# zrc0622/HIRL4UCAV

Measured on AMD Instinct MI355X. Metric: env steps/sec (whole node) + HIRL update steps/sec at 4096 envs/GPU, higher is better.
Workload: dtype f32

## Files before the change

hirl4ucav_amd/agents/engine.py:

```python
import ctypes
import os

import numpy as np
import torch

from .. import _lib

H1, H2 = 256, 512
_vp, _i32, _f32 = ctypes.c_void_p, ctypes.c_int32, ctypes.c_float


class HxBatch(ctypes.Structure):
    _fields_ = [("rows", _vp), ("bc_rows", _vp), ("batch", _i32), ("noise", _vp)]


class HxSample(ctypes.Structure):
    _fields_ = [("total", _vp), ("cap", ctypes.c_int64), ("ring", _vp), ("expert_ring", _vp), ("expert_len", ctypes.c_int64),
                ("bc_table", _vp), ("bc_len", ctypes.c_int64), ("n_main", _i32), ("seed", ctypes.c_uint64), ("call", ctypes.c_uint32),
                ("sigma", _f32), ("idx", _vp), ("idx_bc", _vp), ("guard", ctypes.c_uint32)]


class HxFront(ctypes.Structure):
    _fields_ = [("flags", _vp), ("status", _vp), ("epoch", ctypes.c_uint32), ("with_c", ctypes.c_uint32)]

# ... 415 lines not shown
        B, st = self.batch, _lib.stream_ptr()
        nets, hyper = ctypes.byref(self.nets), ctypes.byref(self.hyper)
        gs = 1.0 / self.world
        own_critic = self.grad_critic.data_ptr()
        if self.xchg is not None:
            self.nets.grad_critic = self.xchg.write_buffer("critic").data_ptr()
        critic_grads()
        if before_exchange is not None:
            before_exchange()
        summed = self._allreduce(self.grad_critic, "critic")
        self.nets.grad_critic = summed.data_ptr()
        pk = 16 if do_polyak else 0
        _lib.call("hx_adam", nets, hyper, 0 | pk, self.critic_step, gs, 0, 0.0, 0.0, B, st)
        self.nets.grad_critic = own_critic
        if actor_phase:
            _lib.call("hx_hirl_actor_backward", nets, ctypes.byref(batch), hyper, int(w_kind == 1), 1, st)
            if self.world > 1 or self.sharded_sequence:
                if self.actor_msg is None:
                    self.actor_msg = torch.zeros(int(_lib.load().hx_actor_message_floats()), dtype=torch.float32, device=self.device)
                msg = self.xchg.write_buffer("actor") if self.xchg is not None else self.actor_msg
                _lib.call("hx_hirl_actor_wgrad_split", nets, hyper, B, msg.data_ptr(), st)
                summed = self._allreduce(msg, "actor")
                _lib.call("hx_adam_mixed", nets, hyper, int(do_polyak), self.actor_step, gs, w_kind, w_given, float(bc_warm_up_weight),
                          B * self.world, summed.data_ptr(), st)
            else:
                _lib.call("hx_hirl_actor_wgrad", nets, hyper, B, B, w_kind, w_given, float(bc_warm_up_weight), st)
                _lib.call("hx_adam", nets, hyper, 1 | pk, self.actor_step, gs, w_kind, w_given, float(bc_warm_up_weight), B, st)

    def step_learn(self, env, expert=None, bc_table=None, n_main=None, act_noise=None, act_sigma=0.0, act_seed=0, out=None, sample_seed=0,
                   smooth_sigma=0.2, bc_weight_now=0.0, bc_warm_up_weight=0.0):
        replay, n, B = env.replay, env.n, self.batch
# ... 68 lines not shown
        knob = os.environ.get("HX_FRONT_C")
        carries_c = knob == "1" or (bool(with_c) and knob != "0")
        if carries_c:
            self._front_c_epoch += 1
        front = HxFront(flags.data_ptr(), status.data_ptr(), self._front_epoch, self._front_c_epoch if carries_c else 0)
        _lib.call("hx_hirl_front", env.state.data_ptr(), n, env.pitch, env.obs.data_ptr(), out.data_ptr(), mode | (32 if (not bf16 and self._x9_for(n, front=True)) else 0),
                  _lib.ptr(act_noise), float(act_sigma), int(act_seed), int(env.env_id0), self.act_calls, env.reward.data_ptr(), env.done.data_ptr(),
                  env.success.data_ptr(), ctypes.byref(env._opts), nets, ctypes.byref(batch), hyper, int(actor_phase), w_kind, ctypes.byref(front), st)
        self._front_enqueued = True
        env.steps_issued += 1
        nxt_draw, nxt_tiles = draw(nxt, self.sample_calls + 1), tiles_of(nxt)
        if not self.staged:
            _lib.call("hx_hirl_learn_back", nets, ctypes.byref(batch), hyper, self.critic_step, int(actor_phase), self.actor_step, int(do_polyak), w_kind, w_given,
                      float(bc_warm_up_weight), ctypes.byref(nxt_draw), ctypes.byref(nxt_tiles), with_c, st)
        else:
            self._learn_staged(lambda: _lib.call("hx_hirl_critic_grads_back", nets, ctypes.byref(batch), hyper, ctypes.byref(nxt_draw), ctypes.byref(nxt_tiles), with_c, st),
                               batch, actor_phase, do_polyak, w_kind, w_given, bc_warm_up_weight)
        self._front_drawn = (env, env.steps_issued, replay, expert, bc_table, n_main, int(sample_seed), float(smooth_sigma), self.sample_calls + 1, n)
        self._front_tiles = [nxt, cur]
        self.rows, self.bc_rows, self._idx, self._idx_bc, self._noise = cur
        self.actor_trainable = not self.actor_trainable
        return out, env.obs, env.reward, env.done, env.success

    @staticmethod
    def front_waiting_workgroups(batch, with_c=False):
        tiles = (int(batch) + 15) // 16
        return 2 * tiles * 8 + (2 * ((int(batch) + 7) // 8) * 8 if with_c else 0)

    def front_c_for(self, n, actor_phase, w_kind, bf16):
        if self.front_c != "auto":
            return bool(self.front_c)
# ... 34 lines not shown
```

hirl4ucav_amd/csrc/hx_fwd_body.h:

```cpp
#pragma once
#include "hx_update.h"

namespace hxu {

struct FwdJobC {
    const float* net; const float* src; const float* noise; const float* prev_net;
    float* ws; float* prev_ws;
    uint32_t cfg;
    int32_t rows;
    float noise_clamp;
    float slope;
};
static_assert(sizeof(FwdJobC) == 64, "one s_load_dwordx16");
struct FwdArgsC {
    FwdJobC job[6];
    float slope;
    int zero_nf;
    float* zero_f;
    int* zero_i;
    const uint16_t* images;
    int rowmap;
};
inline FwdJobC pack_fwd(const FwdJob& J) {
    FwdJobC c{};
// ... 72 lines not shown
    const int in = J.m.in;
    constexpr int TPC = WIDE ? 16 : kWide / NT;
    constexpr int NW2 = WIDE ? 1 : H1 / (TPC * 4);
    v4f w2v[NW2];
    uint4 bq[BF16 ? NSL : 1];
    const int lr = lane & 15, lg = lane >> 4, u = wave * 16 + lr;
    STAMP_DECL;
    STAMP();
    const float4* W1v = reinterpret_cast<const float4*>(J.net + J.m.W1());
    const int n4 = H1 * in / 4;
    const float4 wv0 = tid < n4 ? W1v[tid] : make_float4(0.f, 0.f, 0.f, 0.f);
    const float4 wv1 = tid + kWide < n4 ? W1v[tid + kWide] : make_float4(0.f, 0.f, 0.f, 0.f);
    const float bias1 = J.net[J.m.b1() + u], g1v = J.net[J.m.g1() + u], be1v = J.net[J.m.be1() + u];
    const float bias2 = J.net[J.m.b2() + nt * NTW + (WIDE ? wave * 16 : (wave % CT) * 16) + (lane & 15)];
    const int xr = tid / XP, xc = tid % XP;
    const bool head_mode = in == 17 && J.act_mode != 0 && J.act_mode != 3;
    float xv = 0.0f;
    float4 tile_piece = make_float4(0.f, 0.f, 0.f, 0.f);
    if constexpr (SAMPLE) {
        draw_fused(SA, J.rows, s_hkey, s_hown, s_fin);
        if (tid < RT * XP && xr < nrow) {
            const int r = r0 + xr;
            const float* row = (r < SA.n_main ? SA.ring : SA.expert_ring) + (size_t)s_fin[0][r] * 32;
            if (xc < 13) xv = row[J.col0 + xc];
            else if (in == 17 && xc < 17 && J.act_mode == 0) xv = row[xc];
        }
        if (by == 0 && nt < 2 && tid < nrow * 8) {
            const int r = r0 + (tid >> 3);
            if (nt == 0) tile_piece = reinterpret_cast<const float4*>((r < SA.n_main ? SA.ring : SA.expert_ring) + (size_t)s_fin[0][r] * 32)[tid & 7];
            else if (SA.bc_rows) tile_piece = reinterpret_cast<const float4*>(SA.bc_table + (size_t)s_fin[1][r] * 32)[tid & 7];
        }
    } else if (tid < RT * XP && xr < nrow) {
        if (xc < 13) xv = src_row(J.src, r0 + xr)[J.col0 + xc];
        else if (in == 17 && xc < 17) {
            if (J.act_mode == 0) xv = src_row(J.src, r0 + xr)[xc];
            else if (J.act_mode == 3) xv = J.noise[(size_t)(r0 + xr) * 4 + (xc - 13)];
        }
    }
    if constexpr (BF16) {
        const int ctile = WIDE ? nt * 16 + wave : nt * CT + wave % CT;
        const int sl0 = WIDE ? 0 : (wave / CT) * NSL;
        const uint16_t* blk = A.images + (size_t)J.img * kImgElems + (size_t)(ctile * 8 + sl0) * 512 + lane * 8;
#pragma unroll
        for (int i = 0; i < NSL; ++i) bq[i] = *reinterpret_cast<const uint4*>(blk + i * 512);
    } else if (!WIDE) {
        const float* wcol = J.net + J.m.W2() + (size_t)(nt * NT + tid / TPC) * H1 + (tid % TPC) * 4;
#pragma unroll
        for (int i = 0; i < NW2; ++i) w2v[i] = *reinterpret_cast<const v4f*>(wcol + i * TPC * 4);
    }
    STAMP();
    if constexpr (FRONT == 2) {
// ... 1 lines not shown
            if (tid == 0) {
                int spins = 0;
                while ((int)(__hip_atomic_load(&X.flags[rt], __ATOMIC_RELAXED, __HIP_MEMORY_SCOPE_AGENT) - X.target) < 0) {
                    if (++spins > 4000000) { atomicOr(X.status, 1u); break; }
                    __builtin_amdgcn_s_sleep(1);
                }
            }
            __syncthreads();
            if (tid < nrow * 4) xs[(tid >> 2) * XP + 13 + (tid & 3)] = ld_agent(J.prev.ws.outv + (size_t)(r0 + (tid >> 2)) * OW + (tid & 3));
        }
    }
    if (FRONT != 2 && head_mode && wave < nrow) {
        const int r = wave;
        RowReg<H2> xh, y;
        float mean, rstd, o[4];
        if (J.prev.m.out == 4) head_row4<RELU>(J.prev.ws.z2 + (size_t)(r0 + r) * H2, J.prev.net, J.prev.m, slope, xh, y, mean, rstd, o);
        else head_row<4, RELU>(J.prev.ws.z2 + (size_t)(r0 + r) * H2, J.prev.net, J.prev.m, slope, xh, y, mean, rstd, o);
        if (lane < 4) {
            float a = fast_tanh(lane == 0 ? o[0] : lane == 1 ? o[1] : lane == 2 ? o[2] : o[3]);
            if (J.noise) {
                const float e = fminf(fmaxf(J.noise[lane], -J.noise_clamp), J.noise_clamp);
                a = fminf(fmaxf(a + e, -1.0f), 1.0f);
            }
            xs[r * XP + 13 + lane] = a;
            if (nt == 0) J.prev.ws.outv[(size_t)(r0 + r) * OW + lane] = a;
        }
        if (nt == 0 && lane == 0) {
            J.prev.ws.st2[(size_t)(r0 + r) * 2] = mean;
            J.prev.ws.st2[(size_t)(r0 + r) * 2 + 1] = rstd;
        }
    }
// ... 161 lines not shown
            if (tid == 0) __hip_atomic_fetch_add(&X.flags[(FRONT == 1 ? 16 * by : 48) + rt], 1u, __ATOMIC_RELAXED, __HIP_MEMORY_SCOPE_AGENT);
        }
    }
    if constexpr (FRONT == 1) {
        if (by == 0) {
            __builtin_amdgcn_s_waitcnt(0);
            __syncthreads();
            int* last = reinterpret_cast<int*>(lds);
            if (tid == 0) *last = __hip_atomic_fetch_add(&X.flags[rt], 1u, __ATOMIC_RELAXED, __HIP_MEMORY_SCOPE_AGENT) + 1u == X.arrive;
            __syncthreads();
            if (*last) {
                if (wave < nrow) {
                    const int r = wave;
                    RowReg<H2> xh, y;
                    float mean, rstd, o[4];
                    if (J.m.out == 4) head_row4<RELU, true>(J.ws.z2 + (size_t)(r0 + r) * H2, J.net, J.m, slope, xh, y, mean, rstd, o);
                    else head_row<4, RELU, true>(J.ws.z2 + (size_t)(r0 + r) * H2, J.net, J.m, slope, xh, y, mean, rstd, o);
                    if (lane < 4) {
                        float a = fast_tanh(lane == 0 ? o[0] : lane == 1 ? o[1] : lane == 2 ? o[2] : o[3]);
                        if (X.noise) {
                            const float e = fminf(fmaxf(X.noise[lane], -X.noise_clamp), X.noise_clamp);
                            a = fminf(fmaxf(a + e, -1.0f), 1.0f);
                        }
                        st_agent(&J.ws.outv[(size_t)(r0 + r) * OW + lane], a);
                    }
                    if (lane == 0) {
                        J.ws.st2[(size_t)(r0 + r) * 2] = mean;
                        J.ws.st2[(size_t)(r0 + r) * 2 + 1] = rstd;
                    }
                }
                __builtin_amdgcn_s_waitcnt(0);
// ... 13 lines not shown
```

hirl4ucav_amd/csrc/hx_hirl.hip:

```cpp
#include <cmath>

#include "hx_act.h"

using namespace hxnn;
using namespace hxu;

extern "C" {

int hx_actor_param_count(void) { return kActor.size(); }
int hx_critic_param_count(void) { return 2 * kQ.padded(); }
int64_t hx_hirl_workspace_floats(int32_t batch) { return (int64_t)S_COUNT * kSlotFloats * batch + 64; }
int64_t hx_actor_message_floats(void) { return 2 * (int64_t)kActor.padded() + 64; }
int64_t hx_bf16_images_elems(void) { return (int64_t)IM_COUNT * (int64_t)kImgElems; }

int hx_pack_update_images(const HxNets* N, void* stream) {
    HX_REQUIRE(N && N->w2_bf16_all && (reinterpret_cast<uintptr_t>(N->w2_bf16_all) & 15u) == 0, "hx_pack_update_images: w2_bf16_all must be a 16-byte aligned buffer");
    HX_REQUIRE(N->actor && N->critic && N->target_actor && N->target_critic, "hx_pack_update_images: null network");
    hipStream_t st = (hipStream_t)stream;
    uint16_t* im = N->w2_bf16_all;
    launch_pack_bf16(N->actor + kActor.W2(), im + IM_ACTOR * kImgElems, false, st);
    launch_pack_bf16(N->actor + kActor.W2(), im + IM_ACTOR_T * kImgElems, true, st);
    launch_pack_bf16(N->target_actor + kActor.W2(), im + IM_TA * kImgElems, false, st);
    if (N->bc_actor) launch_pack_bf16(N->bc_actor + kActor.W2(), im + IM_BC * kImgElems, false, st);
    for (int h = 0; h < 2; ++h) {
// ... 72 lines not shown
    G = BwdArgs{};
    G.njobs = 2; G.slope = Hy->slope; G.inv_batch = 1.0f / B; G.losses = N->losses; G.soft_count = N->soft_count;
    for (int h = 0; h < 2; ++h) {
        BwdJob& J = G.job[h];
        J = BwdJob{};
        J.net = N->critic + h * mQ.padded(); J.m = mQ; J.ws = s[S_C1 + h]; J.rows = B; J.mode = BM_CRITIC_TD;
        J.t1 = Head{tc1, mQ, s[S_TC1]}; J.t2 = Head{tc2, mQ, s[S_TC2]}; J.src = src; J.gamma = Hy->gamma;
        J.img_t = IM_C1_T + h;
    }
    G.images = N->w2_bf16_all;
}
static bool front_has_c(bool asked) {
    static const int force = getenv("HX_FRONT_C") ? atoi(getenv("HX_FRONT_C")) : -1;
    return force < 0 ? asked : force != 0;
}
static int critic_back(const HxNets* N, const HxBatch* Bt, const HxHyper* Hy, void* stream, int adam_step, bool polyak, const SampleDev* predraw = nullptr, bool skip_c = false) {
    hipStream_t st = (hipStream_t)stream;
    const Mlp mQ{17, 1, Hy->no_layernorm ? 1 : 0};
    const int B = Bt->batch;
    Slot s[S_COUNT];
    make_slots(N, B, s);
    if (!skip_c) {
        BwdArgs G;
        make_launch_c(N, Bt, Hy, G);
        launch_bwd(0, G, st);
    }
    {
        WgArgs W{};
        W.njobs = 2; W.slope = Hy->slope; W.w_kind = 0; W.w_given = 0.f; W.inv_batch = 1.0f / B;
        W.soft_count = N->soft_count; W.wstate = N->wstate;
        for (int h = 0; h < 2; ++h) {
            WgJob& J = W.job[h];
            J = WgJob{};
            J.net = N->critic + h * mQ.padded(); J.grad = N->grad_critic + h * mQ.padded(); J.m = mQ;
            J.ws[0] = s[S_C1 + h]; J.rows[0] = B; J.nslots = 1; J.wmode[0] = 0;
            if (adam_step > 0) {
                J.p = N->critic + h * mQ.padded();
                J.mom = N->m_critic + h * mQ.padded(); J.var = N->v_critic + h * mQ.padded();
                J.target = polyak ? N->target_critic + h * mQ.padded() : nullptr;
                if (uint16_t* im = N->w2_bf16_all) {
                    J.w2b = im + (IM_C1 + h) * kImgElems; J.w2tb = im + (IM_C1_T + h) * kImgElems; J.tgt_w2b = im + (IM_TC1 + h) * kImgElems;
                }
            }
        }
        W.bf16 = N->w2_bf16_all != nullptr;
        W.predraw = predraw; W.predraw_batch = B;
        if (adam_step > 0) {
            W.ad = make_adam(N, Hy, Hy->lr_critic, adam_step, false);
            launch_wg(W, true, st);
        } else {
            launch_wg(W, false, st);
        }
    }
    HX_CHECK_LAUNCH("hx_hirl_critic_grads");
    return 0;
}
static int critic_grads_impl(const HxNets* N, const HxBatch* Bt, const HxHyper* Hy, int32_t actor_fwd, void* stream, int adam_step, bool polyak,
                             const HxSample* S = nullptr) {
    HX_REQUIRE(N && Bt && Hy && Bt->batch > 0 && Bt->batch % 16 == 0, "hx_hirl_critic_grads: batch must be a positive multiple of 16");
    hipStream_t st = (hipStream_t)stream;
    const int B = Bt->batch;
    SampleDev SD{};
    bool fused = false;
    if (S) {
        HX_REQUIRE(Bt->noise, "hx_hirl_*_sampled: the draw needs the output word noise[4]");
        if (int rc = prepare_draw(S, B, const_cast<float*>(Bt->rows), const_cast<float*>(Bt->bc_rows), const_cast<float*>(Bt->noise), stream, &SD, &fused)) return rc;
    }
    FwdArgs F;
    make_launch_a(N, Bt, Hy, actor_fwd, F);
    F.sample = fused ? &SD : nullptr;
    launch_fwd(F, st);
    make_launch_b(N, Bt, Hy, actor_fwd, F);
    launch_fwd(F, st);
    return critic_back(N, Bt, Hy, stream, adam_step, polyak);
}
int hx_hirl_critic_grads(const HxNets* N, const HxBatch* Bt, const HxHyper* Hy, int32_t actor_fwd, void* stream) {
    return critic_grads_impl(N, Bt, Hy, actor_fwd, stream, 0, false);
}
int hx_hirl_critic_grads_sampled(const HxNets* N, const HxBatch* Bt, const HxHyper* Hy, const HxSample* S, int32_t actor_fwd, void* stream) {
    HX_REQUIRE(S, "hx_hirl_critic_grads_sampled: null sample description");
    return critic_grads_impl(N, Bt, Hy, actor_fwd, stream, 0, false, S);
}

int hx_hirl_actor_backward(const HxNets* N, const HxBatch* Bt, const HxHyper* Hy, int32_t estimate_soft, int32_t fwd_done, void* stream) {
    HX_REQUIRE(N && Bt && Hy && Bt->batch > 0 && Bt->batch % 16 == 0, "hx_hirl_actor_backward: batch must be a positive multiple of 16");
    hipStream_t st = (hipStream_t)stream;
    const Mlp mA{13, 4, Hy->no_layernorm ? 1 : 0}, mQ{17, 1, Hy->no_layernorm ? 1 : 0};
    (void)mA; (void)mQ;
    const int B = Bt->batch;
    Slot s[S_COUNT];
    make_slots(N, B, s);
    const RowSrc src{Bt->rows, nullptr, nullptr, 0, 32};
    const RowSrc bcsrc{Bt->bc_rows ? Bt->bc_rows : Bt->rows, nullptr, nullptr, 0, 32};
    const bool bc = Hy->use_bc != 0, soft = bc && estimate_soft;
    if (!fwd_done) {
        FwdArgs F{};
        F.slope = Hy->slope;
        F.zero_f = N->losses + 1; F.zero_nf = 4; F.zero_i = N->soft_count;
        int n = 0;
        F.job[n++] = FwdJob{N->actor, mA, src, 0, 0, Head{}, nullptr, 0.f, s[S_API], B, 1, IM_ACTOR};
        if (bc) F.job[n++] = FwdJob{N->actor, mA, bcsrc, 0, 0, Head{}, nullptr, 0.f, s[S_ABC], B, 1, IM_ACTOR};
        if (soft) F.job[n++] = FwdJob{N->bc_actor, mA, src, 0, 0, Head{}, nullptr, 0.f, s[S_BCS], B, 0, IM_BC};
        F.njobs = n;
        F.images = N->w2_bf16_all;
        launch_fwd(F, st);
    }
    {
        FwdArgs F{};
        F.slope = Hy->slope;
        int n = 0;
        F.job[n++] = FwdJob{N->critic, mQ, src, 0, 1, Head{N->actor, mA, s[S_API]}, nullptr, 0.f, s[S_CPI], B, 1, IM_C1};
        if (soft) F.job[n++] = FwdJob{N->critic, mQ, src, 0, 1, Head{N->bc_actor, mA, s[S_BCS]}, nullptr, 0.f, s[S_CSOFT], B, 0, IM_C1};
        F.njobs = n;
        F.images = N->w2_bf16_all;
        launch_fwd(F, st);
    }
    {
        BwdArgs G{};
        G.njobs = 1; G.slope = Hy->slope; G.inv_batch = 1.0f / B; G.losses = N->losses; G.soft_count = N->soft_count;
        BwdJob& J = G.job[0];
        J = BwdJob{};
        J.net = N->critic; J.m = mQ; J.ws = s[S_CPI]; J.rows = B; J.mode = BM_CRITIC_PI;
        if (soft) J.soft = Head{N->critic, mQ, s[S_CSOFT]};
        J.img_t = IM_C1_T;
        G.images = N->w2_bf16_all;
        launch_bwd(1, G, st);
    }
// ... 88 lines not shown
    W.count_out = msg + 2 * mA.padded();
    launch_wg(W, false, (hipStream_t)stream);
    HX_CHECK_LAUNCH("hx_hirl_actor_wgrad_split");
    return 0;
}

int hx_hirl_learn(const HxNets* N, const HxBatch* Bt, const HxHyper* Hy, int32_t critic_step, int32_t actor_phase,
                  int32_t actor_step, int32_t do_polyak, int32_t w_kind, float w_given, float warm, void* stream) {
    return hx_hirl_learn_sampled(N, Bt, Hy, nullptr, critic_step, actor_phase, actor_step, do_polyak, w_kind, w_given, warm, stream);
}
int hx_hirl_learn_sampled(const HxNets* N, const HxBatch* Bt, const HxHyper* Hy, const HxSample* S, int32_t critic_step, int32_t actor_phase,
                          int32_t actor_step, int32_t do_polyak, int32_t w_kind, float w_given, float warm, void* stream) {
    HX_REQUIRE(critic_step >= 1 && (!actor_phase || actor_step >= 1), "hx_hirl_learn: Adam steps are 1-based");
    int rc = critic_grads_impl(N, Bt, Hy, actor_phase ? (w_kind == 1 ? 2 : 1) : 0, stream, critic_step, do_polyak != 0, S);
    if (rc || !actor_phase) return rc;
    if ((rc = hx_hirl_actor_backward(N, Bt, Hy, w_kind == 1, 1, stream))) return rc;
    return actor_wgrad_impl(N, Hy, Bt->batch, Bt->batch, w_kind, w_given, warm, stream, actor_step, do_polyak != 0);
}

int hx_hirl_front(float* state, int64_t n, int64_t stride, float* obs_io, float* actions, int32_t noise_mode, const float* noise,
                  float sigma, uint64_t seed, uint32_t row0, uint32_t call, float* reward, uint8_t* done, int8_t* success, const HxStepOpts* opts,
                  const HxNets* N, const HxBatch* Bt, const HxHyper* Hy, int32_t actor_phase, int32_t w_kind, const HxFront* front, void* stream) {
    HX_REQUIRE(N && Bt && Hy && front && opts && Bt->batch > 0 && Bt->batch % 16 == 0 && Bt->batch <= kFusedBatchMax && Bt->rows && Bt->noise,
               "hx_hirl_front: the minibatch tiles (a positive multiple of 16 rows, at most 256) and noise[4] must be there");
    HX_REQUIRE(front->flags && front->status && front->epoch >= 1, "hx_hirl_front: flags, status and a 1-based epoch are required");
    const bool bf16 = N->w2_bf16_all != nullptr;
    HX_REQUIRE(bf16 ? N->actor_w2_bf16 != nullptr : (!N->actor_w2_bf16 && (N->actor_w2_f32i || N->actor_w2_x9)),
               "hx_hirl_front: fp32 networks with HxNets.actor_w2_f32i / actor_w2_x9, or the bf16 update path (w2_bf16_all) with actor_w2_bf16");
    const int actor_fwd = actor_phase ? (w_kind == 1 ? 2 : 1) : 0;
    FwdArgs FA, FB;
    make_launch_a(N, Bt, Hy, actor_fwd, FA);
// ... 13 lines not shown
                        *front, (hipStream_t)stream);
}
static int make_predraw(const HxNets* N, const HxBatch* Bt, const HxSample* next, const HxBatch* next_tiles, void* stream, SampleDev* SD) {
    HX_REQUIRE(next_tiles && next_tiles->batch == Bt->batch && next_tiles->rows && next_tiles->noise && next_tiles->rows != Bt->rows && next_tiles->noise != Bt->noise,
               "hx_hirl_learn_back: the next minibatch needs tiles of its own (this call still reads the current ones)");
    (void)N;
    bool fused = false;
    if (int rc = prepare_draw(next, Bt->batch, const_cast<float*>(next_tiles->rows), const_cast<float*>(next_tiles->bc_rows), const_cast<float*>(next_tiles->noise),
                              stream, SD, &fused, false)) return rc;
    HX_REQUIRE(fused, "hx_hirl_learn_back: the predraw covers minibatches of at most 256 rows");
    return 0;
}
int hx_hirl_critic_grads_back(const HxNets* N, const HxBatch* Bt, const HxHyper* Hy, const HxSample* next, const HxBatch* next_tiles, int32_t c_in_front,
                              void* stream) {
    HX_REQUIRE(N && Bt && Hy && Bt->batch > 0 && Bt->batch % 16 == 0, "hx_hirl_critic_grads_back: batch must be a positive multiple of 16");
    SampleDev SD{};
    if (next) if (int rc = make_predraw(N, Bt, next, next_tiles, stream, &SD)) return rc;
    return critic_back(N, Bt, Hy, stream, 0, false, next ? &SD : nullptr, front_has_c(c_in_front != 0));
}
int hx_hirl_learn_back(const HxNets* N, const HxBatch* Bt, const HxHyper* Hy, int32_t critic_step, int32_t actor_phase, int32_t actor_step, int32_t do_polyak,
                       int32_t w_kind, float w_given, float warm, const HxSample* next, const HxBatch* next_tiles, int32_t c_in_front, void* stream) {
    HX_REQUIRE(N && Bt && Hy && Bt->batch > 0 && Bt->batch % 16 == 0, "hx_hirl_learn_back: batch must be a positive multiple of 16");
    HX_REQUIRE(critic_step >= 1 && (!actor_phase || actor_step >= 1), "hx_hirl_learn_back: Adam steps are 1-based");
    SampleDev SD{};
    if (next) if (int rc = make_predraw(N, Bt, next, next_tiles, stream, &SD)) return rc;
    int rc = critic_back(N, Bt, Hy, stream, critic_step, do_polyak != 0, next ? &SD : nullptr, front_has_c(c_in_front != 0));
    if (rc || !actor_phase) return rc;
    if ((rc = hx_hirl_actor_backward(N, Bt, Hy, w_kind == 1, 1, stream))) return rc;
    return actor_wgrad_impl(N, Hy, Bt->batch, Bt->batch, w_kind, w_given, warm, stream, actor_step, do_polyak != 0);
}

int hx_bc_train_actor(const HxNets* N, const HxBatch* Bt, const HxHyper* Hy, int32_t step, void* stream) {
    HX_REQUIRE(N && Bt && Hy && Bt->bc_rows && Bt->batch > 0 && Bt->batch % 16 == 0 && step >= 1, "hx_bc_train_actor: bad arguments");
    hipStream_t st = (hipStream_t)stream;
    const Mlp mA{13, 4, Hy->no_layernorm ? 1 : 0}, mQ{17, 1, Hy->no_layernorm ? 1 : 0};
    (void)mA; (void)mQ;
    const int B = Bt->batch;
    Slot s[S_COUNT];
    make_slots(N, B, s);
    const RowSrc bcsrc{Bt->bc_rows, nullptr, nullptr, 0, 32};
    {
        FwdArgs F{};
        F.njobs = 1; F.slope = Hy->slope;
// ... 31 lines not shown
```

hirl4ucav_amd/csrc/hx_update.h:

```cpp
#pragma once
#include <cmath>
#include <cstdlib>
#include <type_traits>

#include "hx_common.h"
#include "hx_nn.h"

#ifdef HX_STAMPS
static __device__ float hx_dbg[80];
#define STAMP_DECL unsigned long long TS_[16]; int tsn_ = 0
#define STAMP() TS_[tsn_++] = __builtin_amdgcn_s_memrealtime()
#define STAMP_FLUSH(base, cond) do { if (cond) { for (int i_ = 1; i_ < tsn_; ++i_) hx_dbg[(base) + i_] = (float)(TS_[i_] - TS_[i_ - 1]); hx_dbg[(base)] = (float)tsn_; } } while (0)
constexpr int kSpanCap = 8192;
static __device__ unsigned long long hx_span[kSpanCap][2];
static __device__ unsigned hx_span_tag[kSpanCap];
static __device__ unsigned hx_span_n;
#define SPAN_LOG(tag) do { if (threadIdx.x == 0) { const unsigned long long e_ = __builtin_amdgcn_s_memrealtime(); const unsigned i_ = atomicAdd(&hx_span_n, 1u); \
    if (i_ < (unsigned)kSpanCap) { hx_span[i_][0] = TS_[0]; hx_span[i_][1] = e_; hx_span_tag[i_] = (unsigned)(tag) | (blockIdx.x << 8) | (blockIdx.y << 24); } } } while (0)
#define HX_DEFINE_DEBUG_COLLECTORS(name, lo, hi) \
    namespace hx { \
    int dbg_stamps_##name(float* host80) { \
        float tmp[80]; \
        if (hipMemcpyFromSymbol(tmp, HIP_SYMBOL(hx_dbg), sizeof(tmp)) != hipSuccess) return -2; \
        for (int i = (lo); i < (hi); ++i) host80[i] = tmp[i]; \
// ... 127 lines not shown
    }
#pragma unroll
    for (int j = 0; j < OUTMAX; ++j) {
        float acc = 0.0f;
        if (j < m.out) {
            RowReg<H2> w;
            w.load(net + m.W3() + j * H2);
#pragma unroll
            for (int i = 0; i < 8; ++i) acc += act_f<RELU>(y.v[i], slope) * w.v[i];
            acc = wave_sum(acc) + net[m.b3() + j];
        }
        o[j] = acc;
    }
}

template <bool RELU, bool AGENT = false>
__device__ __forceinline__ void head_row4(const float* __restrict__ z2row, const float* __restrict__ net, const Mlp m, float slope,
                                          RowReg<H2>& xhat, RowReg<H2>& y, float& mean, float& rstd, float (&o)[4]) {
    RowReg<H2> z, g, be, w0, w1, w2, w3;
    if (AGENT) z.load_agent(z2row);
    else z.load(z2row);
    g.load(net + m.g2());
    be.load(net + m.be2());
    w0.load(net + m.W3());
    w1.load(net + m.W3() + H2);
    w2.load(net + m.W3() + 2 * H2);
    w3.load(net + m.W3() + 3 * H2);
    const int lane = threadIdx.x & 63;
    const float b3 = net[m.b3() + (lane & 3)];
    row_stats<8>(z.v, H2, mean, rstd);
    if (m.no_ln) { mean = 0.0f; rstd = 1.0f; }
    float a0 = 0.f, a1 = 0.f, a2 = 0.f, a3 = 0.f;
#pragma unroll
    for (int i = 0; i < 8; ++i) {
        xhat.v[i] = (z.v[i] - mean) * rstd;
        y.v[i] = g.v[i] * xhat.v[i] + be.v[i];
    }
#pragma unroll
    for (int i = 0; i < 8; ++i) a0 += act_f<RELU>(y.v[i], slope) * w0.v[i];
#pragma unroll
    for (int i = 0; i < 8; ++i) a1 += act_f<RELU>(y.v[i], slope) * w1.v[i];
#pragma unroll
    for (int i = 0; i < 8; ++i) a2 += act_f<RELU>(y.v[i], slope) * w2.v[i];
#pragma unroll
    for (int i = 0; i < 8; ++i) a3 += act_f<RELU>(y.v[i], slope) * w3.v[i];
    o[0] = wave_sum(a0) + __shfl(b3, 0);
    o[1] = wave_sum(a1) + __shfl(b3, 1);
    o[2] = wave_sum(a2) + __shfl(b3, 2);
    o[3] = wave_sum(a3) + __shfl(b3, 3);
}

__device__ __forceinline__ void philox4x32_10(uint32_t c0, uint32_t c1, uint32_t c2, uint32_t c3, uint32_t k0, uint32_t k1, uint32_t out[4]) {
#pragma unroll
    for (int r = 0; r < 10; ++r) {
        const uint32_t h0 = __umulhi(0xD2511F53u, c0), l0 = 0xD2511F53u * c0;
        const uint32_t h1 = __umulhi(0xCD9E8D57u, c2), l1 = 0xCD9E8D57u * c2;
        const uint32_t n0 = h1 ^ c1 ^ k0, n2 = h0 ^ c3 ^ k1;
        c0 = n0; c1 = l1; c2 = n2; c3 = l0;
        k0 += 0x9E3779B9u; k1 += 0xBB67AE85u;
    }
// ... 330 lines not shown
    float target_entropy, alpha_step_size;
};
struct WgArgs {
    WgJob job[2];
    int njobs;
    float slope;
    WgAdam ad;
    int w_kind;
    float w_given, warm, inv_batch;
    const int* soft_count;
    const float* wstate;
    int bf16;
    float* count_out;
    const SampleDev* predraw;
    int predraw_batch;
};

#pragma clang fp contract(off)
__device__ __forceinline__ void adam_update(float& p, float& m, float& v, float g, float b1, float b2, float eps, float step_size, float bc2_sqrt) {
    m = __builtin_fmaf(g, 1.0f - b1, m * b1);
    v = __builtin_fmaf(g * g, 1.0f - b2, v * b2);
    const float denom = __builtin_amdgcn_sqrtf(v) * __builtin_amdgcn_rcpf(bc2_sqrt) + eps;
    p = p - step_size * (m * __builtin_amdgcn_rcpf(denom));
}
__device__ __forceinline__ float polyak_update(float target, float p, float tau) { return target * (1.0f - tau) + p * tau; }
#pragma clang fp contract(fast)
__device__ __forceinline__ void sac_alpha_step(float* alpha_state, float* losses, float mean_h, float te, float b1, float b2, float eps, float step_size,
                                               float bc2_sqrt) {
    float la = alpha_state[0], m = alpha_state[1], v = alpha_state[2];
    losses[3] = -(la * (te - mean_h));
    adam_update(la, m, v, mean_h - te, b1, b2, eps, step_size, bc2_sqrt);
// ... 202 lines not shown
```

hirl4ucav_amd/csrc/hx_wgrad.hip:

```cpp
#include <cmath>

#include "hx_update.h"

using namespace hxnn;
using namespace hxu;

namespace {

struct WgJobC {
    const float* net; float* grad;
    float* ws0; float* ws1;
    float* mom; float* var; float* target; uint16_t* w2b; float* w2f;
    uint32_t cfg;
    int32_t rows0, rows1;
    float slope, w_given, warm, inv_batch;
    float b1, b2, eps, step_size, bc2_sqrt, tau;
    uint32_t pad_;
    const int* soft_count; float* wstate; float* losses;
    uint16_t* w2tb; uint16_t* tgt_w2b;
    float* count_out;
};
static_assert(sizeof(WgJobC) == 176, "WgJobC layout");
struct WgArgsC {
    WgJobC job[2];
    int has_pre, pre_batch;
    SampleDev pre;
};

struct AdamElem {
    float p, m, v, t;
    __device__ __forceinline__ void fetch(const WgJob& J, unsigned idx) {
        p = J.p[idx];
        m = J.mom[idx];
        v = J.var[idx];
        t = J.target ? J.target[idx] : 0.0f;
    }
    __device__ __forceinline__ void apply(const WgJob& J, const WgAdam& a, unsigned idx, float g) {
        adam_update(p, m, v, g, a.b1, a.b2, a.eps, a.step_size, a.bc2_sqrt);
        J.p[idx] = p;
// ... 169 lines not shown
    const float xh = (z - ri.x) * ri.y;
    const float dy = act_bwd<RELU>(d, g1 * xh + be1, slope);
    const float dz = sc * (ri.y * (dy * g1 - ri.z - xh * ri.w));
    a.db1 += dz;
    a.dbe += sc * dy;
    a.dg += sc * dy * xh;
    const float4* xr4 = reinterpret_cast<const float4*>(xrow);
#pragma unroll
    for (int q = 0; q < 4; ++q) {
        const float4 x4 = xr4[q];
        a.dw1[4 * q] += dz * x4.x; a.dw1[4 * q + 1] += dz * x4.y; a.dw1[4 * q + 2] += dz * x4.z; a.dw1[4 * q + 3] += dz * x4.w;
    }
    a.dw1[16] += dz * xrow[16];
}

#ifdef HX_STAMPS_L1
#define STAMP_L1() STAMP()
#else
#define STAMP_L1()
#endif
template <bool ADAM, bool RELU, bool BF16 = false>
__global__ __launch_bounds__(kWide) void wgrad_kernel(WgArgsC AC) {
    __shared__ __attribute__((aligned(16))) float lds[kWgRowChunk * XP + kWgRowChunk * 12 + kWgRG * kWgCols * kRedP];
    float* xs = lds;
    float* rinfo = lds + kWgRowChunk * XP;
    float* red = rinfo + kWgRowChunk * 12;

    {
        static_assert(sizeof(lds) >= (4 * kFusedSlots + 2 * kFusedBatchMax) * 4, "predraw_wg's tables fit");
        if (AC.has_pre && blockIdx.x >= kWgPerJob) {
            if (blockIdx.x == kWgPerJob && blockIdx.y == 0) predraw_wg(AC.pre, AC.pre_batch, lds);
            return;
        }
    }
    const int j = blockIdx.y, b = blockIdx.x;
    WgJob J;
    WgArgs A;
    expand_wg(AC.job[j], J, A);
    const int tid = threadIdx.x, wave = tid >> 6, lane = tid & 63;
    const float slope = A.slope;
    STAMP_DECL;
    STAMP();
    const float w = effective_w(A.w_kind, A.w_given, A.warm, A.inv_batch, A.soft_count, A.wstate);
    float scale[2];
#pragma unroll
    for (int s = 0; s < 2; ++s) scale[s] = J.wmode[s] == 0 ? 1.0f : (J.wmode[s] == 1 ? 1.0f - w : w);
// ... 568 lines not shown
        const float4 s4 = *reinterpret_cast<const float4*>(source + i);
        t4.x = polyak_update(t4.x, s4.x, tau);
        t4.y = polyak_update(t4.y, s4.y, tau);
        t4.z = polyak_update(t4.z, s4.z, tau);
        t4.w = polyak_update(t4.w, s4.w, tau);
        *reinterpret_cast<float4*>(target + i) = t4;
        return;
    }
    for (int c = 0; c < n - i; ++c) target[i + c] = polyak_update(target[i + c], source[i + c], tau);
}

}

namespace hxu {

void launch_wg(const WgArgs& W, bool adam, hipStream_t st) {
    WgArgsC C{};
    for (int j = 0; j < W.njobs; ++j) C.job[j] = pack_wg(W.job[j], W);
    const bool pre = W.predraw != nullptr;
    C.has_pre = pre ? 1 : 0;
    if (pre) { C.pre = *W.predraw; C.pre_batch = W.predraw_batch; }
    const dim3 grid(kWgPerJob + (pre ? 8 : 0), W.njobs);
    const bool relu = W.slope == 0.0f;
#define HX_WG(ADAM_, RELU_, BF16_) hipLaunchKernelGGL((wgrad_kernel<ADAM_, RELU_, BF16_>), grid, dim3(kWide), 0, st, C)
    static const int dbg_off = getenv("HX_DBG_BF16_OFF") ? atoi(getenv("HX_DBG_BF16_OFF")) : 0;
    static const bool two_on = !(getenv("HX_WGRAD_TWO_SLOT") && atoi(getenv("HX_WGRAD_TWO_SLOT")) == 0);
    const WgJob& J0 = W.job[0];
    if (W.bf16 && !(dbg_off & 4)) {
        if (adam) { if (relu) HX_WG(true, true, true); else HX_WG(true, false, true); }
        else { if (relu) HX_WG(false, true, true); else HX_WG(false, false, true); }
    } else if (two_on && W.njobs == 1 && J0.nslots == 2 && J0.rows[0] > 0 && J0.rows[1] > 0 && J0.rows[0] + J0.rows[1] <= kWgRowChunk) {
        const dim3 grid2(kWg2PerJob + (pre ? 8 : 0), 1);
#define HX_WG2(ADAM_, RELU_) hipLaunchKernelGGL((wgrad2_kernel<ADAM_, RELU_>), grid2, dim3(kWide), 0, st, C)
        if (adam) { if (relu) HX_WG2(true, true); else HX_WG2(true, false); }
        else { if (relu) HX_WG2(false, true); else HX_WG2(false, false); }
#undef HX_WG2
    } else {
        if (adam) { if (relu) HX_WG(true, true, false); else HX_WG(true, false, false); }
        else { if (relu) HX_WG(false, true, false); else HX_WG(false, false, false); }
    }
#undef HX_WG
}
void launch_adam(const AdamArgs& A, hipStream_t st) {
    hipLaunchKernelGGL(adam_kernel, dim3((A.n / 4 + kThreads) / kThreads), dim3(kThreads), 0, st, A);
}
void launch_polyak(float* target, const float* source, int n, float tau, float* target2, const float* source2, int n2, hipStream_t st, const uint32_t* guard) {
// ... 110 lines not shown
```

Measured before the change: 80.98 million.

## Compute actor head outputs in spare critic wgrad workgroups for actor backward reuse

Extra workgroups appended to the critic weight-gradient launch now compute the actor (and BC actor) output head: LayerNorm, activation, 4-wide output and tanh. They store outputs and LN stats so the later actor backward forward pass can read them (act_mode 2) instead of recomputing the head. A pinned-rounding head_row4 variant makes the rider and the forward path round identically. This takes head work off the serialized actor path, but it enlarges the wgrad grid and disables the two-slot wgrad kernel when heads ride.

```diff
diff --git a/hirl4ucav_amd/agents/engine.py b/hirl4ucav_amd/agents/engine.py
--- a/hirl4ucav_amd/agents/engine.py
+++ b/hirl4ucav_amd/agents/engine.py
@@ -453,7 +453,7 @@
         _lib.call("hx_adam", nets, hyper, 0 | pk, self.critic_step, gs, 0, 0.0, 0.0, B, st)
         self.nets.grad_critic = own_critic
         if actor_phase:
-            _lib.call("hx_hirl_actor_backward", nets, ctypes.byref(batch), hyper, int(w_kind == 1), 1, st)
+            _lib.call("hx_hirl_actor_backward", nets, ctypes.byref(batch), hyper, int(w_kind == 1), 2, st)
             if self.world > 1 or self.sharded_sequence:
                 if self.actor_msg is None:
                     self.actor_msg = torch.zeros(int(_lib.load().hx_actor_message_floats()), dtype=torch.float32, device=self.device)
@@ -552,7 +552,9 @@
             _lib.call("hx_hirl_learn_back", nets, ctypes.byref(batch), hyper, self.critic_step, int(actor_phase), self.actor_step, int(do_polyak), w_kind, w_given,
                       float(bc_warm_up_weight), ctypes.byref(nxt_draw), ctypes.byref(nxt_tiles), with_c, st)
         else:
-            self._learn_staged(lambda: _lib.call("hx_hirl_critic_grads_back", nets, ctypes.byref(batch), hyper, ctypes.byref(nxt_draw), ctypes.byref(nxt_tiles), with_c, st),
+            heads = ((4 if (w_kind == 1 and self.use_bc) else 2) if actor_phase else 0)
+            self._learn_staged(lambda: _lib.call("hx_hirl_critic_grads_back", nets, ctypes.byref(batch), hyper, ctypes.byref(nxt_draw), ctypes.byref(nxt_tiles),
+                                                 with_c | heads, st),
                                batch, actor_phase, do_polyak, w_kind, w_given, bc_warm_up_weight)
         self._front_drawn = (env, env.steps_issued, replay, expert, bc_table, n_main, int(sample_seed), float(smooth_sigma), self.sample_calls + 1, n)
         self._front_tiles = [nxt, cur]
diff --git a/hirl4ucav_amd/csrc/hx_fwd_body.h b/hirl4ucav_amd/csrc/hx_fwd_body.h
--- a/hirl4ucav_amd/csrc/hx_fwd_body.h
+++ b/hirl4ucav_amd/csrc/hx_fwd_body.h
@@ -110,7 +110,7 @@
     const float bias1 = J.net[J.m.b1() + u], g1v = J.net[J.m.g1() + u], be1v = J.net[J.m.be1() + u];
     const float bias2 = J.net[J.m.b2() + nt * NTW + (WIDE ? wave * 16 : (wave % CT) * 16) + (lane & 15)];
     const int xr = tid / XP, xc = tid % XP;
-    const bool head_mode = in == 17 && J.act_mode != 0 && J.act_mode != 3;
+    const bool head_mode = in == 17 && J.act_mode == 1;
     float xv = 0.0f;
     float4 tile_piece = make_float4(0.f, 0.f, 0.f, 0.f);
     if constexpr (SAMPLE) {
@@ -131,6 +131,7 @@
         else if (in == 17 && xc < 17) {
             if (J.act_mode == 0) xv = src_row(J.src, r0 + xr)[xc];
             else if (J.act_mode == 3) xv = J.noise[(size_t)(r0 + xr) * 4 + (xc - 13)];
+            else if (J.act_mode == 2) xv = J.prev.ws.outv[(size_t)(r0 + xr) * OW + (xc - 13)];
         }
     }
     if constexpr (BF16) {
@@ -162,7 +163,7 @@
         const int r = wave;
         RowReg<H2> xh, y;
         float mean, rstd, o[4];
-        if (J.prev.m.out == 4) head_row4<RELU>(J.prev.ws.z2 + (size_t)(r0 + r) * H2, J.prev.net, J.prev.m, slope, xh, y, mean, rstd, o);
+        if (J.prev.m.out == 4) head_row4<RELU, false, true>(J.prev.ws.z2 + (size_t)(r0 + r) * H2, J.prev.net, J.prev.m, slope, xh, y, mean, rstd, o);
         else head_row<4, RELU>(J.prev.ws.z2 + (size_t)(r0 + r) * H2, J.prev.net, J.prev.m, slope, xh, y, mean, rstd, o);
         if (lane < 4) {
             float a = fast_tanh(lane == 0 ? o[0] : lane == 1 ? o[1] : lane == 2 ? o[2] : o[3]);
@@ -354,7 +355,7 @@
                     const int r = wave;
                     RowReg<H2> xh, y;
                     float mean, rstd, o[4];
-                    if (J.m.out == 4) head_row4<RELU, true>(J.ws.z2 + (size_t)(r0 + r) * H2, J.net, J.m, slope, xh, y, mean, rstd, o);
+                    if (J.m.out == 4) head_row4<RELU, true, true>(J.ws.z2 + (size_t)(r0 + r) * H2, J.net, J.m, slope, xh, y, mean, rstd, o);
                     else head_row<4, RELU, true>(J.ws.z2 + (size_t)(r0 + r) * H2, J.net, J.m, slope, xh, y, mean, rstd, o);
                     if (lane < 4) {
                         float a = fast_tanh(lane == 0 ? o[0] : lane == 1 ? o[1] : lane == 2 ? o[2] : o[3]);
diff --git a/hirl4ucav_amd/csrc/hx_hirl.hip b/hirl4ucav_amd/csrc/hx_hirl.hip
--- a/hirl4ucav_amd/csrc/hx_hirl.hip
+++ b/hirl4ucav_amd/csrc/hx_hirl.hip
@@ -110,7 +110,9 @@
     static const int force = getenv("HX_FRONT_C") ? atoi(getenv("HX_FRONT_C")) : -1;
     return force < 0 ? asked : force != 0;
 }
-static int critic_back(const HxNets* N, const HxBatch* Bt, const HxHyper* Hy, void* stream, int adam_step, bool polyak, const SampleDev* predraw = nullptr, bool skip_c = false) {
+static int heads_of(const HxHyper* Hy, int actor_fwd) { return actor_fwd ? ((actor_fwd == 2 && Hy->use_bc) ? 2 : 1) : 0; }
+static int critic_back(const HxNets* N, const HxBatch* Bt, const HxHyper* Hy, void* stream, int adam_step, bool polyak, int heads, const SampleDev* predraw = nullptr,
+                       bool skip_c = false) {
     hipStream_t st = (hipStream_t)stream;
     const Mlp mQ{17, 1, Hy->no_layernorm ? 1 : 0};
     const int B = Bt->batch;
@@ -141,6 +143,11 @@
         }
         W.bf16 = N->w2_bf16_all != nullptr;
         W.predraw = predraw; W.predraw_batch = B;
+        if (heads && head_rider_on()) {
+            const Mlp mA{13, 4, Hy->no_layernorm ? 1 : 0};
+            W.head[0] = Head{N->actor, mA, s[S_API]}; W.head_rows[0] = B; W.nhead = 1;
+            if (heads == 2) { W.head[1] = Head{N->bc_actor, mA, s[S_BCS]}; W.head_rows[1] = B; W.nhead = 2; }
+        }
         if (adam_step > 0) {
             W.ad = make_adam(N, Hy, Hy->lr_critic, adam_step, false);
             launch_wg(W, true, st);
@@ -168,7 +175,7 @@
     launch_fwd(F, st);
     make_launch_b(N, Bt, Hy, actor_fwd, F);
     launch_fwd(F, st);
-    return critic_back(N, Bt, Hy, stream, adam_step, polyak);
+    return critic_back(N, Bt, Hy, stream, adam_step, polyak, heads_of(Hy, actor_fwd));
 }
 int hx_hirl_critic_grads(const HxNets* N, const HxBatch* Bt, const HxHyper* Hy, int32_t actor_fwd, void* stream) {
     return critic_grads_impl(N, Bt, Hy, actor_fwd, stream, 0, false);
@@ -189,6 +196,7 @@
     const RowSrc src{Bt->rows, nullptr, nullptr, 0, 32};
     const RowSrc bcsrc{Bt->bc_rows ? Bt->bc_rows : Bt->rows, nullptr, nullptr, 0, 32};
     const bool bc = Hy->use_bc != 0, soft = bc && estimate_soft;
+    const int act_g = (fwd_done == 2 && head_rider_on()) ? 2 : 1;
     if (!fwd_done) {
         FwdArgs F{};
         F.slope = Hy->slope;
@@ -205,8 +213,8 @@
         FwdArgs F{};
         F.slope = Hy->slope;
         int n = 0;
-        F.job[n++] = FwdJob{N->critic, mQ, src, 0, 1, Head{N->actor, mA, s[S_API]}, nullptr, 0.f, s[S_CPI], B, 1, IM_C1};
-        if (soft) F.job[n++] = FwdJob{N->critic, mQ, src, 0, 1, Head{N->bc_actor, mA, s[S_BCS]}, nullptr, 0.f, s[S_CSOFT], B, 0, IM_C1};
+        F.job[n++] = FwdJob{N->critic, mQ, src, 0, act_g, Head{N->actor, mA, s[S_API]}, nullptr, 0.f, s[S_CPI], B, 1, IM_C1};
+        if (soft) F.job[n++] = FwdJob{N->critic, mQ, src, 0, act_g, Head{N->bc_actor, mA, s[S_BCS]}, nullptr, 0.f, s[S_CSOFT], B, 0, IM_C1};
         F.njobs = n;
         F.images = N->w2_bf16_all;
         launch_fwd(F, st);
@@ -325,7 +333,7 @@
     HX_REQUIRE(critic_step >= 1 && (!actor_phase || actor_step >= 1), "hx_hirl_learn: Adam steps are 1-based");
     int rc = critic_grads_impl(N, Bt, Hy, actor_phase ? (w_kind == 1 ? 2 : 1) : 0, stream, critic_step, do_polyak != 0, S);
     if (rc || !actor_phase) return rc;
-    if ((rc = hx_hirl_actor_backward(N, Bt, Hy, w_kind == 1, 1, stream))) return rc;
+    if ((rc = hx_hirl_actor_backward(N, Bt, Hy, w_kind == 1, 2, stream))) return rc;
     return actor_wgrad_impl(N, Hy, Bt->batch, Bt->batch, w_kind, w_given, warm, stream, actor_step, do_polyak != 0);
 }
 
@@ -369,9 +377,11 @@
 int hx_hirl_critic_grads_back(const HxNets* N, const HxBatch* Bt, const HxHyper* Hy, const HxSample* next, const HxBatch* next_tiles, int32_t c_in_front,
                               void* stream) {
     HX_REQUIRE(N && Bt && Hy && Bt->batch > 0 && Bt->batch % 16 == 0, "hx_hirl_critic_grads_back: batch must be a positive multiple of 16");
+    HX_REQUIRE(c_in_front >= 0 && c_in_front < 6 && (c_in_front < 4 || (Hy->use_bc && N->bc_actor)),
+               "hx_hirl_critic_grads_back: c_in_front is 0 / 1 (+ 2: actor(s)'s head rides, + 4: bc_actor(s)'s too — a BC agent's soft-estimate call)");
     SampleDev SD{};
     if (next) if (int rc = make_predraw(N, Bt, next, next_tiles, stream, &SD)) return rc;
-    return critic_back(N, Bt, Hy, stream, 0, false, next ? &SD : nullptr, front_has_c(c_in_front != 0));
+    return critic_back(N, Bt, Hy, stream, 0, false, (c_in_front >> 1) & 3, next ? &SD : nullptr, front_has_c((c_in_front & 1) != 0));
 }
 int hx_hirl_learn_back(const HxNets* N, const HxBatch* Bt, const HxHyper* Hy, int32_t critic_step, int32_t actor_phase, int32_t actor_step, int32_t do_polyak,
                        int32_t w_kind, float w_given, float warm, const HxSample* next, const HxBatch* next_tiles, int32_t c_in_front, void* stream) {
@@ -379,9 +389,10 @@
     HX_REQUIRE(critic_step >= 1 && (!actor_phase || actor_step >= 1), "hx_hirl_learn_back: Adam steps are 1-based");
     SampleDev SD{};
     if (next) if (int rc = make_predraw(N, Bt, next, next_tiles, stream, &SD)) return rc;
-    int rc = critic_back(N, Bt, Hy, stream, critic_step, do_polyak != 0, next ? &SD : nullptr, front_has_c(c_in_front != 0));
+    int rc = critic_back(N, Bt, Hy, stream, critic_step, do_polyak != 0, heads_of(Hy, actor_phase ? (w_kind == 1 ? 2 : 1) : 0), next ? &SD : nullptr,
+                         front_has_c(c_in_front != 0));
     if (rc || !actor_phase) return rc;
-    if ((rc = hx_hirl_actor_backward(N, Bt, Hy, w_kind == 1, 1, stream))) return rc;
+    if ((rc = hx_hirl_actor_backward(N, Bt, Hy, w_kind == 1, 2, stream))) return rc;
     return actor_wgrad_impl(N, Hy, Bt->batch, Bt->batch, w_kind, w_given, warm, stream, actor_step, do_polyak != 0);
 }
 
diff --git a/hirl4ucav_amd/csrc/hx_update.h b/hirl4ucav_amd/csrc/hx_update.h
--- a/hirl4ucav_amd/csrc/hx_update.h
+++ b/hirl4ucav_amd/csrc/hx_update.h
@@ -165,7 +165,30 @@
     }
 }
 
-template <bool RELU, bool AGENT = false>
+#pragma clang fp contract(off)
+__device__ __forceinline__ float head_dot8(const float (&h)[8], const float (&w)[8]) {
+    float a = __builtin_fmaf(h[0], w[0], 0.0f);
+    a = __builtin_fmaf(h[1], w[1], a);
+#pragma unroll
+    for (int i = 2; i < 8; ++i) {
+        const float p = h[i] * w[i];
+        a = a + p;
+    }
+    return a;
+}
+__device__ __forceinline__ float head_var8(const float (&d)[8]) {
+    const float p1 = d[1] * d[1];
+    float q = __builtin_fmaf(d[0], d[0], p1);
+#pragma unroll
+    for (int i = 2; i < 8; ++i) {
+        const float p = d[i] * d[i];
+        q = q + p;
+    }
+    return q;
+}
+#pragma clang fp contract(fast)
+
+template <bool RELU, bool AGENT = false, bool PIN = false>
 __device__ __forceinline__ void head_row4(const float* __restrict__ z2row, const float* __restrict__ net, const Mlp m, float slope,
                                           RowReg<H2>& xhat, RowReg<H2>& y, float& mean, float& rstd, float (&o)[4]) {
     RowReg<H2> z, g, be, w0, w1, w2, w3;
@@ -179,22 +202,40 @@
     w3.load(net + m.W3() + 3 * H2);
     const int lane = threadIdx.x & 63;
     const float b3 = net[m.b3() + (lane & 3)];
-    row_stats<8>(z.v, H2, mean, rstd);
-    if (m.no_ln) { mean = 0.0f; rstd = 1.0f; }
     float a0 = 0.f, a1 = 0.f, a2 = 0.f, a3 = 0.f;
-#pragma unroll
-    for (int i = 0; i < 8; ++i) {
-        xhat.v[i] = (z.v[i] - mean) * rstd;
-        y.v[i] = g.v[i] * xhat.v[i] + be.v[i];
-    }
-#pragma unroll
-    for (int i = 0; i < 8; ++i) a0 += act_f<RELU>(y.v[i], slope) * w0.v[i];
-#pragma unroll
-    for (int i = 0; i < 8; ++i) a1 += act_f<RELU>(y.v[i], slope) * w1.v[i];
-#pragma unroll
-    for (int i = 0; i < 8; ++i) a2 += act_f<RELU>(y.v[i], slope) * w2.v[i];
-#pragma unroll
-    for (int i = 0; i < 8; ++i) a3 += act_f<RELU>(y.v[i], slope) * w3.v[i];
+    if constexpr (PIN) {
+        float s = 0.0f, d[8], h[8];
+#pragma unroll
+        for (int i = 0; i < 8; ++i) s += z.v[i];
+        mean = wave_sum(s) / (float)H2;
+#pragma unroll
+        for (int i = 0; i < 8; ++i) d[i] = z.v[i] - mean;
+        rstd = __builtin_amdgcn_rsqf(wave_sum(head_var8(d)) / (float)H2 + LN_EPS);
+        if (m.no_ln) { mean = 0.0f; rstd = 1.0f; }
+#pragma unroll
+        for (int i = 0; i < 8; ++i) {
+            xhat.v[i] = (z.v[i] - mean) * rstd;
+            y.v[i] = __builtin_fmaf(g.v[i], xhat.v[i], be.v[i]);
+            h[i] = act_f<RELU>(y.v[i], slope);
+        }
+        a0 = head_dot8(h, w0.v); a1 = head_dot8(h, w1.v); a2 = head_dot8(h, w2.v); a3 = head_dot8(h, w3.v);
+    } else {
+        row_stats<8>(z.v, H2, mean, rstd);
+        if (m.no_ln) { mean = 0.0f; rstd = 1.0f; }
+#pragma unroll
+        for (int i = 0; i < 8; ++i) {
+            xhat.v[i] = (z.v[i] - mean) * rstd;
+            y.v[i] = g.v[i] * xhat.v[i] + be.v[i];
+        }
+#pragma unroll
+        for (int i = 0; i < 8; ++i) a0 += act_f<RELU>(y.v[i], slope) * w0.v[i];
+#pragma unroll
+        for (int i = 0; i < 8; ++i) a1 += act_f<RELU>(y.v[i], slope) * w1.v[i];
+#pragma unroll
+        for (int i = 0; i < 8; ++i) a2 += act_f<RELU>(y.v[i], slope) * w2.v[i];
+#pragma unroll
+        for (int i = 0; i < 8; ++i) a3 += act_f<RELU>(y.v[i], slope) * w3.v[i];
+    }
     o[0] = wave_sum(a0) + __shfl(b3, 0);
     o[1] = wave_sum(a1) + __shfl(b3, 1);
     o[2] = wave_sum(a2) + __shfl(b3, 2);
@@ -555,7 +596,11 @@
     float* count_out;
     const SampleDev* predraw;
     int predraw_batch;
-};
+    Head head[2];
+    int head_rows[2];
+    int nhead;
+};
+bool head_rider_on();
 
 #pragma clang fp contract(off)
 __device__ __forceinline__ void adam_update(float& p, float& m, float& v, float g, float b1, float b2, float eps, float step_size, float bc2_sqrt) {
diff --git a/hirl4ucav_amd/csrc/hx_wgrad.hip b/hirl4ucav_amd/csrc/hx_wgrad.hip
--- a/hirl4ucav_amd/csrc/hx_wgrad.hip
+++ b/hirl4ucav_amd/csrc/hx_wgrad.hip
@@ -21,8 +21,14 @@
     float* count_out;
 };
 static_assert(sizeof(WgJobC) == 176, "WgJobC layout");
+struct HeadJobC {
+    const float* net; float* ws;
+    int32_t rows;
+    uint32_t cfg;
+};
 struct WgArgsC {
     WgJobC job[2];
+    HeadJobC head[2];
     int has_pre, pre_batch;
     SampleDev pre;
 };
@@ -222,6 +228,40 @@
     a.dw1[16] += dz * xrow[16];
 }
 
+__device__ __forceinline__ int extra_slot() {
+    const int c = (int)blockIdx.x - kWgPerJob;
+    return ((c >> 3) * (int)gridDim.y + (int)blockIdx.y) * 8 + (c & 7);
+}
+inline int extra_columns(int slots, int njobs) { return 8 * ((slots + 8 * njobs - 1) / (8 * njobs)); }
+template <bool RELU>
+__device__ __forceinline__ void head_rider_wg(const WgArgsC& AC, int t) {
+    if (t < 0) return;
+    const float slope = AC.job[0].slope;
+    const int wave = (int)threadIdx.x >> 6, lane = (int)threadIdx.x & 63;
+#pragma unroll
+    for (int h = 0; h < 2; ++h) {
+        const HeadJobC& hj = AC.head[h];
+        const int tiles = (hj.rows + RT - 1) / RT;
+        if (t < tiles) {
+            const int r = t * RT + wave;
+            if (r >= hj.rows) return;
+            const Mlp m = mlp_of(hj.cfg & 1023u);
+            const Slot S = carve_slot(hj.ws, hj.rows);
+            RowReg<H2> xh, y;
+            float mean, rstd, o[4];
+            if (m.out == 4) head_row4<RELU, false, true>(S.z2 + (size_t)r * H2, hj.net, m, slope, xh, y, mean, rstd, o);
+            else head_row<4, RELU>(S.z2 + (size_t)r * H2, hj.net, m, slope, xh, y, mean, rstd, o);
+            if (lane < 4) S.outv[(size_t)r * OW + lane] = fast_tanh(lane == 0 ? o[0] : lane == 1 ? o[1] : lane == 2 ? o[2] : o[3]);
+            if (lane == 0) {
+                S.st2[(size_t)r * 2] = mean;
+                S.st2[(size_t)r * 2 + 1] = rstd;
+            }
+            return;
+        }
+        t -= tiles;
+    }
+}
+
 #ifdef HX_STAMPS_L1
 #define STAMP_L1() STAMP()
 #else
@@ -236,8 +276,10 @@
 
     {
         static_assert(sizeof(lds) >= (4 * kFusedSlots + 2 * kFusedBatchMax) * 4, "predraw_wg's tables fit");
-        if (AC.has_pre && blockIdx.x >= kWgPerJob) {
-            if (blockIdx.x == kWgPerJob && blockIdx.y == 0) predraw_wg(AC.pre, AC.pre_batch, lds);
+        if (blockIdx.x >= kWgPerJob) {
+            const int s = extra_slot();
+            if (AC.has_pre && s == 0) predraw_wg(AC.pre, AC.pre_batch, lds);
+            else head_rider_wg<RELU>(AC, s - (AC.has_pre ? 8 : 0));
             return;
         }
     }
@@ -836,13 +878,24 @@
 
 namespace hxu {
 
+bool head_rider_on() {
+    static const bool on = !(getenv("HX_HEAD_RIDER") && atoi(getenv("HX_HEAD_RIDER")) == 0);
+    return on;
+}
+
 void launch_wg(const WgArgs& W, bool adam, hipStream_t st) {
     WgArgsC C{};
     for (int j = 0; j < W.njobs; ++j) C.job[j] = pack_wg(W.job[j], W);
     const bool pre = W.predraw != nullptr;
     C.has_pre = pre ? 1 : 0;
     if (pre) { C.pre = *W.predraw; C.pre_batch = W.predraw_batch; }
-    const dim3 grid(kWgPerJob + (pre ? 8 : 0), W.njobs);
+    int head_tiles = 0;
+    for (int h = 0; h < W.nhead && h < 2; ++h) {
+        C.head[h] = HeadJobC{W.head[h].net, W.head[h].ws.x, W.head_rows[h], mlp_bits(W.head[h].m)};
+        head_tiles += (W.head_rows[h] + RT - 1) / RT;
+    }
+    const int extra = (pre || head_tiles) ? extra_columns((pre ? 8 : 0) + head_tiles, W.njobs) : 0;
+    const dim3 grid(kWgPerJob + extra, W.njobs);
     const bool relu = W.slope == 0.0f;
 #define HX_WG(ADAM_, RELU_, BF16_) hipLaunchKernelGGL((wgrad_kernel<ADAM_, RELU_, BF16_>), grid, dim3(kWide), 0, st, C)
     static const int dbg_off = getenv("HX_DBG_BF16_OFF") ? atoi(getenv("HX_DBG_BF16_OFF")) : 0;
@@ -851,7 +904,7 @@
     if (W.bf16 && !(dbg_off & 4)) {
         if (adam) { if (relu) HX_WG(true, true, true); else HX_WG(true, false, true); }
         else { if (relu) HX_WG(false, true, true); else HX_WG(false, false, true); }
-    } else if (two_on && W.njobs == 1 && J0.nslots == 2 && J0.rows[0] > 0 && J0.rows[1] > 0 && J0.rows[0] + J0.rows[1] <= kWgRowChunk) {
+    } else if (two_on && head_tiles == 0 && W.njobs == 1 && J0.nslots == 2 && J0.rows[0] > 0 && J0.rows[1] > 0 && J0.rows[0] + J0.rows[1] <= kWgRowChunk) {
         const dim3 grid2(kWg2PerJob + (pre ? 8 : 0), 1);
 #define HX_WG2(ADAM_, RELU_) hipLaunchKernelGGL((wgrad2_kernel<ADAM_, RELU_>), grid2, dim3(kWide), 0, st, C)
         if (adam) { if (relu) HX_WG2(true, true); else HX_WG2(true, false); }
```

New measurement: 83.04 million, median of 6. +2.5%, better.
